# leggedrobotics/wild_visual_navigation

Measured on NVIDIA H100. Metric: frames/sec end-to-end (DINO feat + seg + MLP train-step) at 448x448, higher is better.
Workload: dtype bf16 operands / fp32 accumulate (ViT, STEGO head, per-pixel MLP); fp32 (k-means, train step)

## Files before the change

### include/wvn_b200.h

```cpp
#ifndef WVN_B200_H_
#define WVN_B200_H_

#include <stddef.h>
#include <stdint.h>

#ifdef __cplusplus
extern "C" {
#endif

typedef enum {
  WVN_STATUS_OK = 0,
  WVN_STATUS_INVALID = -1,
  WVN_STATUS_CUDA = -2,
  WVN_STATUS_NO_DEVICE = -3,
  WVN_STATUS_STATE = -4
} wvn_status;

const char* wvn_last_error(void);
int wvn_check_device(void);
int wvn_version(void);
long long wvn_launch_count(void);
void wvn_profile_enable(int category_mask);
int wvn_profile_collect(float* host_ms, long long* host_launches);

int wvn_gemm_bf16(const void* a_bf16, long long lda, const void* w_bf16, const float* bias, void* out, long long ldo,
                  int m, int n, int k, int out_kind, int act, int block_n, void* stream);

typedef struct {
  int m, n, k;
  int epi, act;
  int block_n;
  const void* a;
  long long lda;
  const void* w;
  const float* bias;
  void* out;
  long long ldo;
  const float* pos;
  int tokens_in, npad;
  int dim, heads;
  void* q_out;
  void* k_out;
  void* vt_out;
  int feat, trav_col;
  const void* x;
  long long ldx;
  float* trav;
  float* conf;
  float* loss_reco;
  const float* cg_mean;
  const float* cg_std;
  float cg_std_factor;
  int reverse_m;
  int registers;
  const void* residual;
  long long ldr;
} wvn_gemm_ex_args;
int wvn_gemm_bf16_ex(const wvn_gemm_ex_args* args, void* stream);

int wvn_attention_bf16(const void* q, const void* k, const void* vt, void* out, int batch, int heads, int npad,
                       int n_valid, float scale, void* stream);

int wvn_layernorm(const float* x, const float* gamma, const float* beta, void* out_bf16, long long rows, int dim,
                  float eps, void* stream);

typedef struct wvn_vit wvn_vit_t;

typedef struct {
  int image_size;
  int patch_size;
  int dim;
  int depth;
  int heads;
  int mlp_dim;
  int max_batch;
  int chunk;
  float ln_eps;
  int head_out;
  int registers;
} wvn_vit_config;

int wvn_vit_create(const wvn_vit_config* cfg, wvn_vit_t** out);
void wvn_vit_destroy(wvn_vit_t* h);

int wvn_vit_set_weight(wvn_vit_t* h, const char* name, const float* data, long long numel);

int wvn_vit_forward(wvn_vit_t* h, const float* img, int batch, int in_h, int in_w, int resized_h, int resized_w,
                    float* tokens_out, void* stream);

// ... 149 lines not shown
```

### wild_visual_navigation_b200/_C.py

```python
from __future__ import annotations

import ctypes
import os
from ctypes import POINTER, Structure, byref, c_char_p, c_float, c_int, c_longlong, c_size_t, c_void_p

import torch

_HERE = os.path.dirname(os.path.abspath(__file__))
LIB_PATH = os.environ.get("WVN_B200_LIB", os.path.join(_HERE, "libwvn_b200.so"))


class WvnError(RuntimeError):
    pass


class VitConfig(Structure):
    _fields_ = [
        ("image_size", c_int), ("patch_size", c_int), ("dim", c_int), ("depth", c_int), ("heads", c_int),
        ("mlp_dim", c_int), ("max_batch", c_int), ("chunk", c_int), ("ln_eps", c_float), ("head_out", c_int),
        ("registers", c_int),
    ]


class GemmExArgs(Structure):
    _fields_ = [
        ("m", c_int), ("n", c_int), ("k", c_int), ("epi", c_int), ("act", c_int), ("block_n", c_int),
        ("a", c_void_p), ("lda", c_longlong), ("w", c_void_p), ("bias", c_void_p), ("out", c_void_p), ("ldo", c_longlong),
        ("pos", c_void_p), ("tokens_in", c_int), ("npad", c_int), ("dim", c_int), ("heads", c_int),
        ("q_out", c_void_p), ("k_out", c_void_p), ("vt_out", c_void_p),
        ("feat", c_int), ("trav_col", c_int), ("x", c_void_p), ("ldx", c_longlong), ("trav", c_void_p),
        ("conf", c_void_p), ("loss_reco", c_void_p), ("cg_mean", c_void_p), ("cg_std", c_void_p),
        ("cg_std_factor", c_float), ("reverse_m", c_int), ("registers", c_int), ("residual", c_void_p), ("ldr", c_longlong),
    ]


class ResnetConfig(Structure):
    _fields_ = [("image_size", c_int), ("depth", c_int), ("max_batch", c_int)]


class TrainConfig(Structure):
    _fields_ = [
        ("w_trav", c_float), ("w_reco", c_float), ("std_factor", c_float), ("anomaly_balanced", c_int),
        ("lr", c_float), ("beta1", c_float), ("beta2", c_float), ("eps", c_float),
    ]


class FlowBuffers(Structure):
    _fields_ = [("mask0", c_void_p), ("mask1", c_void_p), ("p1", c_void_p), ("invp1", c_void_p), ("p3", c_void_p),
                ("invp3", c_void_p)]


_lib = None

_P, _I, _L, _F, _S = c_void_p, c_int, c_longlong, c_float, c_size_t
SIGNATURES = {
    "wvn_last_error": (c_char_p, []),
    "wvn_check_device": (_I, []),
    "wvn_version": (_I, []),
    "wvn_launch_count": (_L, []),
    "wvn_profile_enable": (None, [_I]),
    "wvn_profile_collect": (_I, [_P, _P]),
    "wvn_gemm_bf16": (_I, [_P, _L, _P, _P, _P, _L, _I, _I, _I, _I, _I, _I, _P]),
    "wvn_gemm_bf16_ex": (_I, [POINTER(GemmExArgs), _P]),
    "wvn_attention_bf16": (_I, [_P, _P, _P, _P, _I, _I, _I, _I, _F, _P]),
    "wvn_layernorm": (_I, [_P, _P, _P, _P, _L, _I, _F, _P]),
# ... 108 lines not shown
```

### wild_visual_navigation_b200/csrc/api.cu

```cuda
#include <cuda_bf16.h>

#include <stdio.h>
#include <stdlib.h>

#include <map>
#include <string>
#include <vector>

#include "../../include/wvn_b200.h"
#include "attention.h"
#include "dense_kernels.h"
#include "gemm.h"
#include "host_common.h"
#include "mlp_train.h"
#include "mlp_train_fused.h"
#include "pixel_head.h"
#include "resnet_kernels.h"
#include "segment_kernels.h"
#include "flow_train.h"
#include "footprint_kernels.h"
#include "slic_kernels.h"
#include "stego_kmeans.h"
#include "train_core.h"
#include "vit_kernels.h"
// ... 54 lines not shown
};

}

struct wvn_vit {
  wvn_vit_config cfg;
  int grid = 0, P = 0, t0 = 1, n_valid = 0, npad = 0, kpe = 0, kpe_ld = 0, chunk = 0;
  std::map<std::string, Weight> w;
  std::vector<DevBuf> owned;
  DevBuf x, xn, q, k, vt, attn, hid, ape, stage;
  DevBuf tok_bf16, head_hidden;
  DevBuf qkv_f32;
  bool precise = false;
  bool forwarded = false;
  int last_batch = 0;

  int add_weight(const std::string& name, long long numel, bool bf16, int cols = 0, int ld = 0) {
    DevBuf b;
    const long long stored = cols > 0 ? numel / cols * ld : numel;
    WVN_PROPAGATE(b.alloc(static_cast<size_t>(stored) * (bf16 ? 2 : 4)));
    owned.push_back(b);
    Weight wt;
    wt.p = b.p; wt.numel = numel; wt.bf16 = bf16; wt.cols = cols; wt.ld = ld;
    w[name] = wt;
    return WVN_OK;
  }
  template <class T>
  T* wp(const std::string& name) { return reinterpret_cast<T*>(w[name].p); }
};

extern "C" {

const char* wvn_last_error(void) { return last_error(); }
int wvn_version(void) { return 104; }

int wvn_check_device(void) {
  int n = 0;
  if (cudaGetDeviceCount(&n) != cudaSuccess || n == 0) return set_error(WVN_ERR_NO_DEVICE, "no CUDA device visible");
  int dev = 0;
  cudaGetDevice(&dev);
  int major = 0;
  cudaDeviceGetAttribute(&major, cudaDevAttrComputeCapabilityMajor, dev);
  int minor = 0;
  cudaDeviceGetAttribute(&minor, cudaDevAttrComputeCapabilityMinor, dev);
  if (major != 9 || minor != 0)
    return set_error(WVN_ERR_NO_DEVICE, "device %d has compute capability %d.%d, need 9.0 (sm_90a)", dev, major, minor);
  return WVN_OK;
}

long long wvn_launch_count(void) { return launch_count(); }
void wvn_profile_enable(int category_mask) { prof_enable(category_mask); }
int wvn_profile_collect(float* host_ms, long long* host_launches) {
  WVN_REQUIRE(host_ms && host_launches, "wvn_profile_collect: null argument");
  return prof_collect(host_ms, host_launches);
}

int wvn_gemm_bf16(const void* a, long long lda, const void* w, const float* bias, void* out, long long ldo, int m, int n,
                  int k, int out_kind, int act, int block_n, void* stream) {
  GemmArgs g;
  g.M = m; g.N = n; g.K = k;
  g.epi = out_kind == 0 ? EPI_BF16 : (out_kind == 1 ? EPI_F32 : EPI_RESID_F32);
  WVN_REQUIRE(out_kind >= 0 && out_kind <= 2, "wvn_gemm_bf16: out_kind %d", out_kind);
  g.act = act; g.bias = bias; g.out = out; g.ldo = ldo;
  return gemm_bf16(g, a, lda, w, block_n, S(stream));
}

int wvn_gemm_bf16_ex(const wvn_gemm_ex_args* x, void* stream) {
  WVN_REQUIRE(x, "wvn_gemm_bf16_ex: null argument");
  GemmArgs g;
  g.M = x->m; g.N = x->n; g.K = x->k; g.epi = x->epi; g.act = x->act;
  g.bias = x->bias; g.out = x->out; g.ldo = x->ldo;
  g.pos = x->pos; g.tokens_in = x->tokens_in; g.npad = x->npad;
  g.dim = x->dim; g.heads = x->heads; g.q = x->q_out; g.k = x->k_out; g.vt = x->vt_out;
  g.feat = x->feat; g.trav_col = x->trav_col; g.x = x->x; g.ldx = x->ldx; g.trav = x->trav; g.conf = x->conf;
  g.loss_reco = x->loss_reco; g.cg_mean = x->cg_mean; g.cg_std = x->cg_std; g.cg_std_factor = x->cg_std_factor;
  g.reverse_m = x->reverse_m; g.registers = x->registers;
  g.residual = x->residual; g.ldr = x->ldr;
  return gemm_bf16(g, x->a, x->lda, x->w, x->block_n, S(stream));
}

int wvn_attention_bf16(const void* q, const void* k, const void* vt, void* out, int batch, int heads, int npad,
                       int n_valid, float scale, void* stream) {
  AttnArgs a;
  a.batch = batch; a.heads = heads; a.npad = npad; a.n_valid = n_valid;
  a.scale_log2 = scale * 1.4426950408889634f;
  a.out = out; a.ldo = static_cast<long long>(heads) * 64;
  return attention_bf16(a, q, k, vt, S(stream));
}

int wvn_layernorm(const float* x, const float* gamma, const float* beta, void* out_bf16, long long rows, int dim,
                  float eps, void* stream) {
  LayerNormArgs a;
  a.rows = rows; a.dim = dim; a.eps = eps;
  return layernorm_rows(x, gamma, beta, out_bf16, nullptr, a, S(stream));
}

int wvn_vit_create(const wvn_vit_config* cfg, wvn_vit_t** out) {
  WVN_REQUIRE(cfg && out, "wvn_vit_create: null argument");
  WVN_PROPAGATE(wvn_check_device());
  WVN_REQUIRE(cfg->dim == 384 || cfg->dim == 768, "vit: dim %d unsupported (384, 768)", cfg->dim);
  WVN_REQUIRE(cfg->heads * 64 == cfg->dim, "vit: heads*64 must equal dim");
  WVN_REQUIRE(cfg->patch_size == 8 || cfg->patch_size == 14 || cfg->patch_size == 16, "vit: patch size %d unsupported",
              cfg->patch_size);
  WVN_REQUIRE(cfg->image_size >= cfg->patch_size, "vit: image size too small");
  WVN_REQUIRE(cfg->mlp_dim % 64 == 0 && cfg->depth > 0 && cfg->max_batch > 0, "vit: bad mlp_dim/depth/max_batch");
  WVN_REQUIRE(cfg->head_out % 64 == 0, "vit: head_out must be a multiple of 64");
  WVN_REQUIRE(cfg->registers >= 0, "vit: registers must be >= 0");
  WVN_REQUIRE(cfg->registers == 0 || cfg->head_out == 0, "vit: register tokens and a STEGO head cannot be combined");
  wvn_vit* h = new wvn_vit();
  h->cfg = *cfg;
// ... 129 lines not shown

static int vit_check_loaded(wvn_vit* h, bool need_head) {
  for (auto& kv : h->w) {
    const bool is_head = kv.first.rfind("stego.", 0) == 0;
    if (is_head && !need_head) continue;
    if (!kv.second.loaded) return set_error(WVN_ERR_STATE, "vit: weight '%s' was never set", kv.first.c_str());
  }
  return WVN_OK;
}

constexpr int kDefaultSubAttn = 1 << 30;

namespace {
int vit_forward_impl(wvn_vit_t* h, const void* img, bool u8_hwc, int batch, int in_h, int in_w, int resized_h, int resized_w,
                     float* tokens_out, void* stream, bool flip_tta = false);
}

int wvn_vit_forward_tta(wvn_vit_t* h, const float* img, int batch, int in_h, int in_w, int resized_h, int resized_w,
                        float* tokens_out, void* stream) {
  return vit_forward_impl(h, img, false, batch, in_h, in_w, resized_h, resized_w, tokens_out, stream, true);
}

int wvn_vit_forward(wvn_vit_t* h, const float* img, int batch, int in_h, int in_w, int resized_h, int resized_w,
                    float* tokens_out, void* stream) {
  return vit_forward_impl(h, img, false, batch, in_h, in_w, resized_h, resized_w, tokens_out, stream);
}

int wvn_vit_forward_u8(wvn_vit_t* h, const unsigned char* img_hwc, int batch, int in_h, int in_w, int resized_h,
                       int resized_w, float* tokens_out, void* stream) {
  return vit_forward_impl(h, img_hwc, true, batch, in_h, in_w, resized_h, resized_w, tokens_out, stream);
}

namespace {
int vit_forward_impl(wvn_vit_t* h, const void* img, bool u8_hwc, int src_batch, int in_h, int in_w, int resized_h, int resized_w,
                     float* tokens_out, void* stream, bool flip_tta) {
  const int batch = flip_tta ? 2 * src_batch : src_batch;
  WVN_REQUIRE(h && img, "wvn_vit_forward: null argument");
  WVN_REQUIRE(batch > 0 && batch <= h->cfg.max_batch, "wvn_vit_forward: batch %d outside (0, %d]", batch, h->cfg.max_batch);
  WVN_REQUIRE(resized_h >= h->cfg.image_size && resized_w >= h->cfg.image_size,
              "wvn_vit_forward: resized image %dx%d smaller than the crop %d", resized_h, resized_w, h->cfg.image_size);
  WVN_PROPAGATE(vit_check_loaded(h, false));
  cudaStream_t s = S(stream);
  const wvn_vit_config& c = h->cfg;
  const int D = c.dim;

  ImagePatchArgs ia;
  ia.in_h = in_h; ia.in_w = in_w; ia.patch = c.patch_size; ia.grid_h = h->grid; ia.grid_w = h->grid;
  ia.crop_top = static_cast<int>(lrintf((resized_h - c.image_size) / 2.0f));
  ia.crop_left = static_cast<int>(lrintf((resized_w - c.image_size) / 2.0f));
  ia.scale_y = static_cast<float>(in_h) / static_cast<float>(resized_h);
  ia.scale_x = static_cast<float>(in_w) / static_cast<float>(resized_w);

  for (int b0 = 0; b0 < batch; b0 += h->chunk) {
    const int nb = std::min(h->chunk, batch - b0);
    const int rows = nb * h->npad;
    float* x = reinterpret_cast<float*>(h->x.p);
    ia.batch = nb;
    ia.frame0 = b0; ia.src_frames = src_batch; ia.flip_from = flip_tta ? src_batch : (1 << 30);
    WVN_PROPAGATE(image_to_patches(img, u8_hwc, h->ape.p, ia, s));
    const float* reg = c.registers > 0 ? h->wp<float>("register_tokens") : nullptr;
    WVN_PROPAGATE(init_token_rows(x, h->wp<float>("cls_token"), h->wp<float>("pos_embed"), reg, c.registers, nb, h->npad,
                                  h->n_valid, D, s));
    {
      GemmArgs g;
      g.M = nb * h->P; g.N = D; g.K = h->kpe; g.epi = EPI_PATCH; g.bias = h->wp<float>("patch_embed.proj.bias");
      g.out = x; g.ldo = D; g.pos = h->wp<float>("pos_embed"); g.tokens_in = h->P; g.npad = h->npad;
      g.registers = c.registers;
      WVN_PROPAGATE(gemm_bf16(g, h->ape.p, h->kpe_ld, h->wp<void>("patch_embed.proj.weight"), 0, s));
    }
    LayerNormArgs la;
    la.rows = rows; la.dim = D; la.eps = c.ln_eps; la.npad = h->npad; la.n_valid = h->n_valid; la.row0 = h->t0;
    static int sub_env = -1;
    if (sub_env < 0) {
      const char* e = getenv("WVN_VIT_SUBCHUNK");
      sub_env = e ? atoi(e) : (1 << 30);
      if (sub_env < 1) sub_env = 1 << 30;
    }
// ... 8 lines not shown
    if (sub_attn_env < 0) {
      const char* e = getenv("WVN_VIT_SUB_ATTN");
      sub_attn_env = e ? atoi(e) : kDefaultSubAttn;
      if (sub_attn_env < 1) sub_attn_env = 1 << 30;
    }
    const int sub_a = std::min(sub_attn_env, nb);
    for (int l = 0; l < c.depth; ++l) {
      const std::string b = "blocks." + std::to_string(l) + ".";
      for (int s0 = 0; s0 < nb; s0 += sub_a) {
        const int ns = std::min(sub_a, nb - s0);
        const long long roff = static_cast<long long>(s0) * h->npad;
        LayerNormArgs ls = la;
        ls.rows = static_cast<long long>(ns) * h->npad;
        ls.reverse = next_dir();
        WVN_PROPAGATE(layernorm_rows(x + roff * D, h->wp<float>(b + "norm1.weight"), h->wp<float>(b + "norm1.bias"),
                                     xn + roff * D, nullptr, ls, s));
        if (h->precise) {
          GemmArgs g;
          float* qkv = reinterpret_cast<float*>(h->qkv_f32.p) + roff * 3 * D;
          g.M = ns * h->npad; g.N = 3 * D; g.K = D; g.epi = EPI_F32; g.bias = h->wp<float>(b + "attn.qkv.bias");
          g.out = qkv; g.ldo = 3 * D;
          WVN_PROPAGATE(gemm_bf16(g, xn + roff * D, D, h->wp<void>(b + "attn.qkv.weight"), 0, s));
          WVN_PROPAGATE(attention_f32_debug(qkv, attn + roff * D, ns, c.heads, h->npad, h->n_valid, D, 0.125f, s));
          continue;
        }
        GemmArgs g;
        g.M = ns * h->npad; g.N = 3 * D; g.K = D; g.epi = EPI_QKV; g.bias = h->wp<float>(b + "attn.qkv.bias");
        g.npad = h->npad; g.dim = D; g.heads = c.heads;
        const long long hoff = static_cast<long long>(s0) * c.heads * h->npad * 64;
        g.q = reinterpret_cast<__nv_bfloat16*>(h->q.p) + hoff;
        g.k = reinterpret_cast<__nv_bfloat16*>(h->k.p) + hoff;
        g.vt = reinterpret_cast<__nv_bfloat16*>(h->vt.p) + hoff;
        g.reverse_m = next_dir();
        WVN_PROPAGATE(gemm_bf16(g, xn + roff * D, D, h->wp<void>(b + "attn.qkv.weight"), 0, s));
        AttnArgs a;
        a.batch = ns; a.heads = c.heads; a.npad = h->npad; a.n_valid = h->n_valid;
        a.scale_log2 = 0.125f * 1.4426950408889634f;
        a.out = attn + roff * D; a.ldo = D;
        a.reverse = next_dir();
        WVN_PROPAGATE(attention_bf16(a, g.q, g.k, g.vt, s));
      }
      for (int s0 = 0; s0 < nb; s0 += sub) {
        const int ns = std::min(sub, nb - s0);
        const long long roff = static_cast<long long>(s0) * h->npad;
        const int srows = ns * h->npad;
        LayerNormArgs ls = la;
        ls.rows = srows;
        {
          GemmArgs g;
          g.M = srows; g.N = D; g.K = D; g.epi = EPI_RESID_F32; g.bias = h->wp<float>(b + "attn.proj.bias");
          g.out = x + roff * D; g.ldo = D;
          g.reverse_m = next_dir();
          WVN_PROPAGATE(gemm_bf16(g, attn + roff * D, D, h->wp<void>(b + "attn.proj.weight"), 0, s));
        }
        ls.reverse = next_dir();
        WVN_PROPAGATE(layernorm_rows(x + roff * D, h->wp<float>(b + "norm2.weight"), h->wp<float>(b + "norm2.bias"),
                                     xn + roff * D, nullptr, ls, s));
        {
          GemmArgs g;
          g.M = srows; g.N = c.mlp_dim; g.K = D; g.epi = EPI_BF16; g.act = ACT_GELU;
          g.bias = h->wp<float>(b + "mlp.fc1.bias"); g.out = h->hid.p; g.ldo = c.mlp_dim;
          g.reverse_m = next_dir();
          WVN_PROPAGATE(gemm_bf16(g, xn + roff * D, D, h->wp<void>(b + "mlp.fc1.weight"), 0, s));
        }
        {
          GemmArgs g;
          g.M = srows; g.N = D; g.K = c.mlp_dim; g.epi = EPI_RESID_F32; g.bias = h->wp<float>(b + "mlp.fc2.bias");
          g.out = x + roff * D; g.ldo = D;
          g.reverse_m = next_dir();
          WVN_PROPAGATE(gemm_bf16(g, h->hid.p, c.mlp_dim, h->wp<void>(b + "mlp.fc2.weight"), 0, s));
        }
      }
    }
    __nv_bfloat16* tok_bf = reinterpret_cast<__nv_bfloat16*>(h->tok_bf16.p) + static_cast<long long>(b0) * h->npad * D;
    float* tok_f = tokens_out ? tokens_out + static_cast<long long>(b0) * h->P * D : nullptr;
    la.reverse = next_dir();
    WVN_PROPAGATE(layernorm_rows(x, h->wp<float>("norm.weight"), h->wp<float>("norm.bias"), tok_bf, tok_f, la, s));
  }
  h->forwarded = true;
  h->last_batch = batch;
  return WVN_OK;
}
}

int wvn_vit_stego_head(wvn_vit_t* h, int batch, float* out, void* stream) {
  WVN_REQUIRE(h && out, "wvn_vit_stego_head: null argument");
  WVN_REQUIRE(h->cfg.head_out > 0, "wvn_vit_stego_head: handle was created without a head");
  WVN_REQUIRE(h->forwarded && batch == h->last_batch, "wvn_vit_stego_head: call wvn_vit_forward with the same batch first");
  WVN_PROPAGATE(vit_check_loaded(h, true));
  cudaStream_t s = S(stream);
  const int D = h->cfg.dim, rows = batch * h->npad, HO = h->cfg.head_out;
  GemmArgs g;
  g.M = rows; g.N = D; g.K = D; g.epi = EPI_BF16; g.act = ACT_RELU; g.bias = h->wp<float>("stego.hidden.bias");
  g.out = h->head_hidden.p; g.ldo = D;
  WVN_PROPAGATE(gemm_bf16(g, h->tok_bf16.p, D, h->wp<void>("stego.hidden.weight"), 0, s));
  GemmArgs a;
  a.M = rows; a.N = HO; a.K = D; a.epi = EPI_F32; a.bias = h->wp<float>("stego.head_a.bias"); a.out = out; a.ldo = HO;
  WVN_PROPAGATE(gemm_bf16(a, h->tok_bf16.p, D, h->wp<void>("stego.head_a.weight"), 0, s));
  GemmArgs b;
  b.M = rows; b.N = HO; b.K = D; b.epi = EPI_RESID_F32; b.bias = nullptr; b.out = out; b.ldo = HO;
  WVN_PROPAGATE(gemm_bf16(b, h->head_hidden.p, D, h->wp<void>("stego.head_b.weight"), 0, s));
  return WVN_OK;
}
// ... 830 lines not shown
```

### wild_visual_navigation_b200/csrc/gemm.h

```cpp
#pragma once

#include <cuda_runtime.h>

namespace wvn {

enum GemmEpilogue : int {
  EPI_BF16 = 0,
  EPI_F32 = 1,
  EPI_RESID_F32 = 2,
  EPI_PATCH = 3,
  EPI_QKV = 4,
  EPI_MLP_HEAD = 5,
  EPI_BF16_RESID = 6,
};

enum GemmAct : int { ACT_NONE = 0, ACT_RELU = 1, ACT_GELU = 2 };

struct GemmArgs {
  int M = 0, N = 0, K = 0;
  int epi = EPI_BF16, act = ACT_NONE;
  const float* bias = nullptr;
  void* out = nullptr;
  long long ldo = 0;
  const float* pos = nullptr;
  int tokens_in = 0;
  int registers = 0;
  int npad = 0;
  int dim = 0, heads = 0;
  void* q = nullptr;
  void* k = nullptr;
  void* vt = nullptr;
  int feat = 0;
  int trav_col = 0;
  const void* x = nullptr;
  long long ldx = 0;
  float* trav = nullptr;
  float* conf = nullptr;
  float* loss_reco = nullptr;
  const float* cg_mean = nullptr;
  const float* cg_std = nullptr;
  float cg_std_factor = 0.5f;
  const void* residual = nullptr;
  long long ldr = 0;
  int max_ctas = 0;
  int reverse_m = 0;
};

int pick_block_n(int N);

inline long long gemm_w_pitch(int K) { return (static_cast<long long>(K) + 7) / 8 * 8; }

int gemm_bf16(const GemmArgs& args, const void* A, long long lda, const void* W, int block_n, cudaStream_t stream);

}
```

### wild_visual_navigation_b200/csrc/gemm_wgmma.cu

```cuda
#include <stdlib.h>

#include <algorithm>

#include "common.cuh"
#include "gemm.h"
#include "host_common.h"

namespace wvn {

namespace {

constexpr int BM = 64;
constexpr int BK = 64;
constexpr int kConsumerWarps = 8;
constexpr int kNumThreads = 128 + kConsumerWarps * 32;
constexpr int kMaxSmemBytes = 227 * 1024;
constexpr int kMaxStages = 8;
constexpr int kFixedSmemBytes = 1024  + 1024 ;
constexpr int kSliceCols = 32;
constexpr int kResidMaxBlockN = 192;

template <bool ROW_OWNER>
struct TileIter {
  int num_m, num_n, m_blk, n_blk, lin;
  __device__ TileIter(int nm, int nn) : num_m(nm), num_n(nn), m_blk(0), n_blk(0), lin(0) {
    if (ROW_OWNER) { m_blk = blockIdx.x; n_blk = 0; }
    else { lin = blockIdx.x; m_blk = lin / num_n; n_blk = lin % num_n; }
  }
  __device__ bool valid() const { return m_blk < num_m; }
  __device__ void next() {
    if (ROW_OWNER) { if (++n_blk == num_n) { n_blk = 0; m_blk += gridDim.x; } }
    else { lin += gridDim.x; m_blk = lin / num_n; n_blk = lin % num_n; }
  }
};

template <int EPI>
constexpr bool kStaged = EPI == EPI_BF16 || EPI == EPI_F32 || EPI == EPI_RESID_F32 || EPI == EPI_QKV || EPI == EPI_BF16_RESID;

template <int BN, int EPI>
struct GemmCfg {
  static constexpr uint32_t kABytes = BM * BK * 2;
  static constexpr uint32_t kBBytes = BN * BK * 2;
  static constexpr uint32_t kStageBytes = kABytes + kBBytes;
  static constexpr uint32_t kSliceBytes = BM * kSliceCols * ((EPI == EPI_F32 || EPI == EPI_RESID_F32) ? 4 : 2);
  static constexpr uint32_t kStagingBytes = kStaged<EPI> ? 2 * 2 * kSliceBytes : 0;
  static constexpr int kStagesRaw = (kMaxSmemBytes - kFixedSmemBytes - kStagingBytes) / kStageBytes;
  static constexpr int kStages = kStagesRaw > kMaxStages ? kMaxStages : kStagesRaw;
  static constexpr uint32_t kSmemBytes = kStages * kStageBytes + kStagingBytes + kFixedSmemBytes;
  static constexpr int kN128 = BN / 128;
  static constexpr int kN64 = (BN % 128) / 64;
  static constexpr int kN32 = (BN % 64) / 32;
};

__device__ __forceinline__ float gelu_erf_fast(float x) {
  const float t = fminf(fabsf(x), 5.5f);
  float p = fmaf(-0.0003865310864f, t, 0.006509808358f);
  p = fmaf(p, t, -0.05048002675f);
  p = fmaf(p, t, -0.4613505006f);
  p = fmaf(p, t, -1.150225043f);
  p = fmaf(p, t, -1.00010848f);
  float e;
  asm("ex2.approx.ftz.f32 %0, %1;" : "=f"(e) : "f"(p));
  return fmaf(-t, e, fmaxf(x, 0.f));
}

template <int ACT>
__device__ __forceinline__ float activate(float v) {
  if (ACT == ACT_RELU) return fmaxf(v, 0.f);
  if (ACT == ACT_GELU) return gelu_erf_fast(v);
  return v;
}

template <int EPI, int ACT, int NREG>
__device__ __forceinline__ void epilogue_frag(const GemmArgs& args, const float (&d)[NREG], const int row0,
// ... 81 lines not shown
        }
        const float v0 = activate<ACT>(a0), v1 = activate<ACT>(a1);
        if (EPI == EPI_F32 || EPI == EPI_RESID_F32) {
          sts64(buf + r * 128 + ((((2 * js + (q >> 1)) ^ (r & 7))) << 4) + (q & 1) * 8, v0, v1);
        } else if (EPI == EPI_QKV && which == 2) {
          const int dd = 8 * js + 2 * q;
          const uint32_t t = 2 * r;
          sts16(buf + dd * 128 + (((t >> 4) ^ (dd & 7)) << 4) + (t & 15), __float2bfloat16_rn(v0));
          sts16(buf + (dd + 1) * 128 + (((t >> 4) ^ ((dd + 1) & 7)) << 4) + (t & 15), __float2bfloat16_rn(v1));
        } else {
          sts32(buf + r * 64 + ((js ^ ((r >> 1) & 3)) << 4) + q * 4, pack_bf16x2(v0, v1));
        }
      }
    }
    fence_proxy_async_smem();
    named_bar_sync(bar_id, 128);
    if (leader) {
      if (EPI == EPI_BF16 || EPI == EPI_F32 || EPI == EPI_BF16_RESID) {
        tma_store_2d(tm0, buf, col, row_tile);
      } else if (EPI == EPI_RESID_F32) {
        tma_reduce_add_2d(tm0, buf, col, row_tile);
      } else if (EPI == EPI_QKV) {
        const int frame = row_tile / args.npad;
        const int tok0 = row_tile - frame * args.npad;
        const int bh = frame * args.heads + (within >> 6);
        if (which < 2) tma_store_2d(which == 0 ? tm0 : tm1, buf, within & 63, bh * args.npad + tok0);
        else tma_store_2d(tm2, buf, tok0, bh * 64 + (within & 63));
      }
      tma_store_commit();
    }
  }
}

template <int BN, int EPI, int ACT>
__global__ void __launch_bounds__(kNumThreads, 1)
gemm_bf16_kernel(const __grid_constant__ CUtensorMap tmap_a, const __grid_constant__ CUtensorMap tmap_b,
                 const __grid_constant__ CUtensorMap tmap_c0, const __grid_constant__ CUtensorMap tmap_c1,
                 const __grid_constant__ CUtensorMap tmap_c2, const GemmArgs args) {
  using Cfg = GemmCfg<BN, EPI>;
  constexpr int STAGES = Cfg::kStages;

  extern __shared__ uint8_t smem_raw[];
  uint8_t* smem = reinterpret_cast<uint8_t*>((reinterpret_cast<uintptr_t>(smem_raw) + 1023) & ~uintptr_t(1023));
  uint8_t* smem_b = smem;
  uint8_t* smem_a = smem + STAGES * Cfg::kBBytes;
  uint8_t* smem_c = smem_a + STAGES * Cfg::kABytes;
  uint64_t* bars = reinterpret_cast<uint64_t*>(smem_c + Cfg::kStagingBytes);
  uint64_t* full_bar = bars;
  uint64_t* empty_bar = bars + kMaxStages;

  const int warp = threadIdx.x >> 5;
  const int lane = threadIdx.x & 31;

  const int num_m = (args.M + BM - 1) / BM;
  const int num_n = args.N / BN;
  const int num_k = (args.K + BK - 1) / BK;
  constexpr bool ROW_OWNER = (EPI == EPI_MLP_HEAD);

  if (threadIdx.x == 0) {
    tma_prefetch_desc(&tmap_a);
    tma_prefetch_desc(&tmap_b);
    for (int i = 0; i < kMaxStages; ++i) {
      mbar_init(&full_bar[i], 1);
      mbar_init(&empty_bar[i], kConsumerWarps / 2);
    }
    fence_mbar_init();
  }
  __syncthreads();

  if (warp < 4) {
    setmaxnreg_dec<40>();
    if (warp == 0) {
      int stage = 0;
      uint32_t phase = 0;
      for (TileIter<ROW_OWNER> it(num_m, num_n); it.valid(); it.next()) {
        const int m_eff = args.reverse_m ? num_m - 1 - it.m_blk : it.m_blk;
        for (int kb = 0; kb < num_k; ++kb) {
          mbar_wait(&empty_bar[stage], phase ^ 1);
          if (elect_one_sync()) {
            mbar_arrive_expect_tx(&full_bar[stage], Cfg::kStageBytes);
            tma_load_2d(&tmap_a, &full_bar[stage], smem_a + stage * Cfg::kABytes, kb * BK, m_eff * BM);
            tma_load_2d(&tmap_b, &full_bar[stage], smem_b + stage * Cfg::kBBytes, kb * BK, it.n_blk * BN);
          }
          __syncwarp();
          if (++stage == STAGES) { stage = 0; phase ^= 1; }
        }
      }
    }
  } else {
    setmaxnreg_inc<232>();
    const int cwarp = warp - 4;
    const int wg = cwarp >> 2;
    const int row_local = (cwarp & 3) * 16 + (lane >> 2);
    const bool leader = (threadIdx.x & 127) == 0;
    const uint32_t staging = smem_u32(smem_c) + wg * 2 * Cfg::kSliceBytes;
    if (kStaged<EPI> && leader) {
      tma_prefetch_desc(&tmap_c0);
      if (EPI == EPI_QKV) {
        tma_prefetch_desc(&tmap_c1);
        tma_prefetch_desc(&tmap_c2);
      }
    }
    if (wg == 1) named_bar_arrive(1, 256);
    float acc128[Cfg::kN128 > 0 ? Cfg::kN128 : 1][64];
    float acc64[32];
    float acc32[16];
    float head_partial[2] = {0.f, 0.f};
    int stage = 0;
    uint32_t phase = 0;
    int unit = 0;
    for (TileIter<ROW_OWNER> it(num_m, num_n); it.valid(); it.next()) {
      const bool unit_end = !ROW_OWNER || it.n_blk == num_n - 1;
      if ((unit & 1) != wg) {
        for (int kb = 0; kb < num_k; ++kb)
          if (++stage == STAGES) { stage = 0; phase ^= 1; }
        if (unit_end) ++unit;
        continue;
      }
      if (!ROW_OWNER || it.n_blk == 0) named_bar_sync(1 + wg, 256);
      int prev_stage = 0;
      for (int kb = 0; kb < num_k; ++kb) {
        mbar_wait(&full_bar[stage], phase);
        const uint64_t desc_a = make_sw128_kmajor_desc(smem_u32(smem_a + stage * Cfg::kABytes));
        const uint32_t b_addr = smem_u32(smem_b + stage * Cfg::kBBytes);
#pragma unroll
        for (int c = 0; c < Cfg::kN128; ++c) wgmma_fence_regs(acc128[c]);
        if (Cfg::kN64) wgmma_fence_regs(acc64);
        if (Cfg::kN32) wgmma_fence_regs(acc32);
        wgmma_fence();
#pragma unroll
        for (int k = 0; k < BK / 16; ++k) {
          const uint32_t accumulate = (kb | k) != 0 ? 1u : 0u;
#pragma unroll
          for (int c = 0; c < Cfg::kN128; ++c)
            wgmma_m64n128k16_ss(acc128[c], desc_a + 2 * k, make_sw128_kmajor_desc(b_addr + c * 128 * 128) + 2 * k, accumulate);
          if (Cfg::kN64)
            wgmma_m64n64k16_ss(acc64, desc_a + 2 * k, make_sw128_kmajor_desc(b_addr + Cfg::kN128 * 128 * 128) + 2 * k, accumulate);
          if (Cfg::kN32)
            wgmma_m64n32k16_ss(acc32, desc_a + 2 * k,
                               make_sw128_kmajor_desc(b_addr + (Cfg::kN128 * 128 + Cfg::kN64 * 64) * 128) + 2 * k, accumulate);
        }
        wgmma_commit();
        if (kb > 0) {
          wgmma_wait<1>();
          if (lane == 0) mbar_arrive(&empty_bar[prev_stage]);
        }
        prev_stage = stage;
        if (++stage == STAGES) { stage = 0; phase ^= 1; }
      }
      if (unit_end && (ROW_OWNER ? it.m_blk + static_cast<int>(gridDim.x) < num_m : it.lin + static_cast<int>(gridDim.x) < num_m * num_n))
        named_bar_arrive(2 - wg, 256);
      wgmma_wait<0>();
#pragma unroll
      for (int c = 0; c < Cfg::kN128; ++c) wgmma_fence_regs(acc128[c]);
      if (Cfg::kN64) wgmma_fence_regs(acc64);
      if (Cfg::kN32) wgmma_fence_regs(acc32);
      if (lane == 0) mbar_arrive(&empty_bar[prev_stage]);

      const int m_eff = args.reverse_m ? num_m - 1 - it.m_blk : it.m_blk;
      const int row_tile = m_eff * BM;
      const int col0 = it.n_blk * BN;
      if (kStaged<EPI>) {
        const int bar_id = 3 + wg;
#pragma unroll
        for (int c = 0; c < Cfg::kN128; ++c)
          store_frag<EPI, ACT>(args, &tmap_c0, &tmap_c1, &tmap_c2, acc128[c], row_tile, col0 + c * 128, row_local, lane,
                               leader, bar_id, staging, Cfg::kSliceBytes, 4 * c);
        if (Cfg::kN64)
          store_frag<EPI, ACT>(args, &tmap_c0, &tmap_c1, &tmap_c2, acc64, row_tile, col0 + Cfg::kN128 * 128, row_local,
                               lane, leader, bar_id, staging, Cfg::kSliceBytes, 4 * Cfg::kN128);
        if (Cfg::kN32)
          store_frag<EPI, ACT>(args, &tmap_c0, &tmap_c1, &tmap_c2, acc32, row_tile, col0 + Cfg::kN128 * 128 + Cfg::kN64 * 64,
                               row_local, lane, leader, bar_id, staging, Cfg::kSliceBytes, 4 * Cfg::kN128 + 2 * Cfg::kN64);
      } else {
        const int row0 = row_tile + row_local;
#pragma unroll
        for (int c = 0; c < Cfg::kN128; ++c)
          epilogue_frag<EPI, ACT>(args, acc128[c], row0, col0 + c * 128, lane, head_partial);
        if (Cfg::kN64) epilogue_frag<EPI, ACT>(args, acc64, row0, col0 + Cfg::kN128 * 128, lane, head_partial);
        if (Cfg::kN32) epilogue_frag<EPI, ACT>(args, acc32, row0, col0 + Cfg::kN128 * 128 + Cfg::kN64 * 64, lane, head_partial);
      }

      if (EPI == EPI_MLP_HEAD && it.n_blk == num_n - 1) {
#pragma unroll
        for (int h = 0; h < 2; ++h) {
          float s = head_partial[h];
          s += __shfl_xor_sync(0xffffffffu, s, 1);
          s += __shfl_xor_sync(0xffffffffu, s, 2);
          head_partial[h] = 0.f;
          const int row = row_tile + row_local + 8 * h;
          if ((lane & 3) == 0 && row < args.M) {
            const float loss = s / static_cast<float>(args.feat);
            const float mean = __ldg(args.cg_mean), sd = __ldg(args.cg_std);
            const float shifted = mean + sd * args.cg_std_factor;
            const float lo = fmaxf(shifted - sd, 0.f);
            const float hi = shifted + sd;
            const float xc = fminf(fmaxf(loss, lo), hi);
            args.conf[row] = 1.f - (xc - lo) / (hi - lo);
            if (args.loss_reco != nullptr) args.loss_reco[row] = loss;
          }
        }
      }
      if (unit_end) ++unit;
    }
    if (kStaged<EPI> && leader) tma_store_wait_all<0>();
  }
}

template <int BN, int EPI, int ACT>
int launch_gemm(const GemmArgs& a, const CUtensorMap& ta, const CUtensorMap& tb, const CUtensorMap (&tc)[3],
                cudaStream_t stream) {
  using Cfg = GemmCfg<BN, EPI>;
  static_assert(Cfg::kStages >= 2, "tile too wide for the shared-memory budget");
  auto kern = gemm_bf16_kernel<BN, EPI, ACT>;
  static bool attr_set = false;
  if (!attr_set) {
    WVN_CHECK_CUDA(cudaFuncSetAttribute(kern, cudaFuncAttributeMaxDynamicSharedMemorySize, kMaxSmemBytes));
    attr_set = true;
  }
  const int num_m = (a.M + BM - 1) / BM, num_n = a.N / BN;
  const int num_tiles = (EPI == EPI_MLP_HEAD) ? num_m : num_m * num_n;
  int grid = sm_count();
  if (a.max_ctas > 0 && a.max_ctas < grid) grid = a.max_ctas;
  if (grid > num_tiles) grid = num_tiles;
  prof_begin(PROF_GEMM, stream);
  kern<<<grid, kNumThreads, Cfg::kSmemBytes, stream>>>(ta, tb, tc[0], tc[1], tc[2], a);
  prof_end(PROF_GEMM, stream);
  WVN_CHECK_LAUNCH("gemm_bf16_kernel");
  return WVN_OK;
}

template <int BN>
int dispatch_epi(const GemmArgs& a, const CUtensorMap& ta, const CUtensorMap& tb, const CUtensorMap (&tc)[3],
                 cudaStream_t s) {
  switch (a.epi) {
    case EPI_BF16:
      if (a.act == ACT_NONE) return launch_gemm<BN, EPI_BF16, ACT_NONE>(a, ta, tb, tc, s);
      if (a.act == ACT_RELU) return launch_gemm<BN, EPI_BF16, ACT_RELU>(a, ta, tb, tc, s);
      if (a.act == ACT_GELU) return launch_gemm<BN, EPI_BF16, ACT_GELU>(a, ta, tb, tc, s);
      break;
    case EPI_F32:
      if (a.act == ACT_NONE) return launch_gemm<BN, EPI_F32, ACT_NONE>(a, ta, tb, tc, s);
      break;
    case EPI_RESID_F32:
      if (a.act == ACT_NONE) return launch_gemm<BN, EPI_RESID_F32, ACT_NONE>(a, ta, tb, tc, s);
      break;
    case EPI_PATCH:
      if (a.act == ACT_NONE) return launch_gemm<BN, EPI_PATCH, ACT_NONE>(a, ta, tb, tc, s);
      break;
    case EPI_QKV:
      if (a.act == ACT_NONE) return launch_gemm<BN, EPI_QKV, ACT_NONE>(a, ta, tb, tc, s);
      break;
    case EPI_MLP_HEAD:
      if (a.act == ACT_NONE) return launch_gemm<BN, EPI_MLP_HEAD, ACT_NONE>(a, ta, tb, tc, s);
      break;
    case EPI_BF16_RESID:
      if constexpr (BN <= kResidMaxBlockN) {
        if (a.act == ACT_NONE) return launch_gemm<BN, EPI_BF16_RESID, ACT_NONE>(a, ta, tb, tc, s);
        if (a.act == ACT_RELU) return launch_gemm<BN, EPI_BF16_RESID, ACT_RELU>(a, ta, tb, tc, s);
      }
      break;
  }
  return set_error(WVN_ERR_INVALID, "gemm: unsupported epilogue/activation combination (%d, %d)", a.epi, a.act);
}

}

int pick_block_n(int N) {
  if (N % 256 == 0) return 256;
  if (N % 224 == 0) return 224;
  if (N % 192 == 0) return 192;
  if (N % 128 == 0) return 128;
  if (N % 64 == 0) return 64;
  return 0;
}

int gemm_bf16(const GemmArgs& a, const void* A, long long lda, const void* W, int block_n, cudaStream_t stream) {
  WVN_REQUIRE(a.M > 0 && a.N > 0 && a.K > 0, "gemm: empty problem (M=%d N=%d K=%d)", a.M, a.N, a.K);
  WVN_REQUIRE(lda >= a.K, "gemm: lda=%lld is smaller than K=%d", lda, a.K);
  if (block_n == 0) {
    block_n = pick_block_n(a.N);
    if (a.epi == EPI_BF16_RESID && block_n > kResidMaxBlockN) block_n = a.N % 192 == 0 ? 192 : (a.N % 128 == 0 ? 128 : 64);
  }
  WVN_REQUIRE(a.epi != EPI_BF16_RESID || block_n <= kResidMaxBlockN, "gemm: the residual epilogue takes block_n <= %d",
              kResidMaxBlockN);
  WVN_REQUIRE(block_n == 64 || block_n == 128 || block_n == 192 || block_n == 224 || block_n == 256,
              "gemm: bad block_n %d", block_n);
  WVN_REQUIRE(a.N % block_n == 0, "gemm: N=%d must be a multiple of block_n=%d (pad the weights)", a.N, block_n);
  if (a.epi == EPI_MLP_HEAD)
    WVN_REQUIRE(a.feat > 0 && a.trav_col % 32 == 0 && a.trav_col >= a.feat && a.trav_col < a.N && a.x != nullptr &&
                    a.trav != nullptr && a.conf != nullptr && a.cg_mean != nullptr && a.cg_std != nullptr &&
                    a.ldx % 8 == 0 && a.ldx >= a.trav_col,
                "gemm: bad MLP-head epilogue arguments (feat=%d trav_col=%d N=%d)", a.feat, a.trav_col, a.N);
  if (a.epi == EPI_QKV)
    WVN_REQUIRE(a.dim % 64 == 0 && a.N == 3 * a.dim && a.heads * 64 == a.dim && a.npad % 8 == 0 && a.npad % BM == 0 &&
                    a.M % a.npad == 0,
                "gemm: bad QKV epilogue geometry (dim=%d heads=%d npad=%d N=%d M=%d)", a.dim, a.heads, a.npad, a.N, a.M);
  if (a.epi == EPI_PATCH)
    WVN_REQUIRE(a.tokens_in > 0 && a.registers >= 0 && 1 + a.registers + a.tokens_in <= a.npad,
                "gemm: bad patch-embed epilogue geometry (tokens_in=%d registers=%d npad=%d)", a.tokens_in, a.registers,
                a.npad);
  if (a.epi == EPI_F32 || a.epi == EPI_RESID_F32) WVN_REQUIRE(a.ldo % 4 == 0, "gemm: fp32 output pitch must be a multiple of 4");
  if (a.epi == EPI_BF16 || a.epi == EPI_BF16_RESID) WVN_REQUIRE(a.ldo % 8 == 0, "gemm: bf16 output pitch must be a multiple of 8");
  if (a.epi == EPI_BF16_RESID)
    WVN_REQUIRE(a.residual != nullptr && a.ldr >= a.N && a.ldr % 2 == 0,
                "gemm: the residual epilogue needs a bf16 residual with an even pitch ldr >= N (ldr=%lld N=%d)", a.ldr, a.N);
  CUtensorMap ta, tb, tc[3] = {};
  WVN_PROPAGATE(make_tmap_bf16_2d(&ta, A, a.K, a.M, static_cast<uint64_t>(lda) * 2, BK, BM));
  WVN_PROPAGATE(make_tmap_bf16_2d(&tb, W, a.K, a.N, static_cast<uint64_t>(gemm_w_pitch(a.K)) * 2, BK, block_n));
  if (a.epi == EPI_BF16 || a.epi == EPI_BF16_RESID)
    WVN_PROPAGATE(make_tmap_2d(&tc[0], a.out, 2, a.N, a.M, static_cast<uint64_t>(a.ldo) * 2, kSliceCols, BM, 64));
  if (a.epi == EPI_F32 || a.epi == EPI_RESID_F32)
    WVN_PROPAGATE(make_tmap_2d(&tc[0], a.out, 4, a.N, a.M, static_cast<uint64_t>(a.ldo) * 4, kSliceCols, BM, 128));
  if (a.epi == EPI_QKV) {
    const uint64_t bh = static_cast<uint64_t>(a.M / a.npad) * a.heads;
    WVN_PROPAGATE(make_tmap_2d(&tc[0], a.q, 2, 64, bh * a.npad, 128, kSliceCols, BM, 64));
    WVN_PROPAGATE(make_tmap_2d(&tc[1], a.k, 2, 64, bh * a.npad, 128, kSliceCols, BM, 64));
    WVN_PROPAGATE(make_tmap_2d(&tc[2], a.vt, 2, a.npad, bh * 64, static_cast<uint64_t>(a.npad) * 2, BM, kSliceCols, 128));
  }
  switch (block_n) {
    case 64: return dispatch_epi<64>(a, ta, tb, tc, stream);
    case 128: return dispatch_epi<128>(a, ta, tb, tc, stream);
    case 192: return dispatch_epi<192>(a, ta, tb, tc, stream);
    case 224: return dispatch_epi<224>(a, ta, tb, tc, stream);
    case 256: return dispatch_epi<256>(a, ta, tb, tc, stream);
  }
  return set_error(WVN_ERR_INVALID, "gemm: unreachable");
}

}
```

Measured before the change: 974.9.

## Add cooperative two-warpgroup GEMM schedule for ViT QKV and MLP projections

Adds a cooperative schedule where both consumer warpgroups share one 2*BM-row tile and a single B tile per stage, instead of ping-pong alternating whole tiles. The ViT QKV, fc1 and fc2 GEMMs now request this schedule with explicit block_n choices. The aim is to halve B-operand traffic per output row and raise arithmetic intensity. In exchange, larger A stages reduce pipeline depth, there are fewer tiles (more wave quantization risk), and the epilogue no longer overlaps with the other warpgroup's mainloop.

```diff
diff --git a/include/wvn_b200.h b/include/wvn_b200.h
--- a/include/wvn_b200.h
+++ b/include/wvn_b200.h
@@ -55,6 +55,7 @@
   int registers;
   const void* residual;
   long long ldr;
+  int schedule;
 } wvn_gemm_ex_args;
 int wvn_gemm_bf16_ex(const wvn_gemm_ex_args* args, void* stream);
 
diff --git a/wild_visual_navigation_b200/_C.py b/wild_visual_navigation_b200/_C.py
--- a/wild_visual_navigation_b200/_C.py
+++ b/wild_visual_navigation_b200/_C.py
@@ -31,6 +31,7 @@
         ("feat", c_int), ("trav_col", c_int), ("x", c_void_p), ("ldx", c_longlong), ("trav", c_void_p),
         ("conf", c_void_p), ("loss_reco", c_void_p), ("cg_mean", c_void_p), ("cg_std", c_void_p),
         ("cg_std_factor", c_float), ("reverse_m", c_int), ("registers", c_int), ("residual", c_void_p), ("ldr", c_longlong),
+        ("schedule", c_int),
     ]
 
 
diff --git a/wild_visual_navigation_b200/csrc/api.cu b/wild_visual_navigation_b200/csrc/api.cu
--- a/wild_visual_navigation_b200/csrc/api.cu
+++ b/wild_visual_navigation_b200/csrc/api.cu
@@ -110,7 +110,7 @@
 extern "C" {
 
 const char* wvn_last_error(void) { return last_error(); }
-int wvn_version(void) { return 104; }
+int wvn_version(void) { return 105; }
 
 int wvn_check_device(void) {
   int n = 0;
@@ -153,7 +153,7 @@
   g.feat = x->feat; g.trav_col = x->trav_col; g.x = x->x; g.ldx = x->ldx; g.trav = x->trav; g.conf = x->conf;
   g.loss_reco = x->loss_reco; g.cg_mean = x->cg_mean; g.cg_std = x->cg_std; g.cg_std_factor = x->cg_std_factor;
   g.reverse_m = x->reverse_m; g.registers = x->registers;
-  g.residual = x->residual; g.ldr = x->ldr;
+  g.residual = x->residual; g.ldr = x->ldr; g.schedule = x->schedule;
   return gemm_bf16(g, x->a, x->lda, x->w, x->block_n, S(stream));
 }
 
@@ -349,6 +349,14 @@
 }
 
 namespace {
+int vit_coop(GemmArgs& g, int preferred) {
+  g.schedule = SCHED_COOP;
+  for (int bn : {preferred, 256, 192, 128})
+    if (g.N % bn == 0) return bn;
+  g.schedule = SCHED_PINGPONG;
+  return 0;
+}
+
 int vit_forward_impl(wvn_vit_t* h, const void* img, bool u8_hwc, int src_batch, int in_h, int in_w, int resized_h, int resized_w,
                      float* tokens_out, void* stream, bool flip_tta) {
   const int batch = flip_tta ? 2 * src_batch : src_batch;
@@ -360,6 +368,7 @@
   cudaStream_t s = S(stream);
   const wvn_vit_config& c = h->cfg;
   const int D = c.dim;
+  const int QKV_BN = 192, FC1_BN = 192, FC2_BN = D <= 384 ? 128 : 256;
 
   ImagePatchArgs ia;
   ia.in_h = in_h; ia.in_w = in_w; ia.patch = c.patch_size; ia.grid_h = h->grid; ia.grid_w = h->grid;
@@ -434,7 +443,8 @@
         g.k = reinterpret_cast<__nv_bfloat16*>(h->k.p) + hoff;
         g.vt = reinterpret_cast<__nv_bfloat16*>(h->vt.p) + hoff;
         g.reverse_m = next_dir();
-        WVN_PROPAGATE(gemm_bf16(g, xn + roff * D, D, h->wp<void>(b + "attn.qkv.weight"), 0, s));
+        const int qkv_bn = vit_coop(g, QKV_BN);
+        WVN_PROPAGATE(gemm_bf16(g, xn + roff * D, D, h->wp<void>(b + "attn.qkv.weight"), qkv_bn, s));
         AttnArgs a;
         a.batch = ns; a.heads = c.heads; a.npad = h->npad; a.n_valid = h->n_valid;
         a.scale_log2 = 0.125f * 1.4426950408889634f;
@@ -463,14 +473,16 @@
           g.M = srows; g.N = c.mlp_dim; g.K = D; g.epi = EPI_BF16; g.act = ACT_GELU;
           g.bias = h->wp<float>(b + "mlp.fc1.bias"); g.out = h->hid.p; g.ldo = c.mlp_dim;
           g.reverse_m = next_dir();
-          WVN_PROPAGATE(gemm_bf16(g, xn + roff * D, D, h->wp<void>(b + "mlp.fc1.weight"), 0, s));
+          const int fc1_bn = vit_coop(g, FC1_BN);
+          WVN_PROPAGATE(gemm_bf16(g, xn + roff * D, D, h->wp<void>(b + "mlp.fc1.weight"), fc1_bn, s));
         }
         {
           GemmArgs g;
           g.M = srows; g.N = D; g.K = c.mlp_dim; g.epi = EPI_RESID_F32; g.bias = h->wp<float>(b + "mlp.fc2.bias");
           g.out = x + roff * D; g.ldo = D;
           g.reverse_m = next_dir();
-          WVN_PROPAGATE(gemm_bf16(g, h->hid.p, c.mlp_dim, h->wp<void>(b + "mlp.fc2.weight"), 0, s));
+          const int fc2_bn = vit_coop(g, FC2_BN);
+          WVN_PROPAGATE(gemm_bf16(g, h->hid.p, c.mlp_dim, h->wp<void>(b + "mlp.fc2.weight"), fc2_bn, s));
         }
       }
     }
diff --git a/wild_visual_navigation_b200/csrc/gemm.h b/wild_visual_navigation_b200/csrc/gemm.h
--- a/wild_visual_navigation_b200/csrc/gemm.h
+++ b/wild_visual_navigation_b200/csrc/gemm.h
@@ -15,6 +15,8 @@
 };
 
 enum GemmAct : int { ACT_NONE = 0, ACT_RELU = 1, ACT_GELU = 2 };
+
+enum GemmSchedule : int { SCHED_PINGPONG = 0, SCHED_COOP = 1 };
 
 struct GemmArgs {
   int M = 0, N = 0, K = 0;
@@ -44,6 +46,7 @@
   long long ldr = 0;
   int max_ctas = 0;
   int reverse_m = 0;
+  int schedule = SCHED_PINGPONG;
 };
 
 int pick_block_n(int N);
diff --git a/wild_visual_navigation_b200/csrc/gemm_wgmma.cu b/wild_visual_navigation_b200/csrc/gemm_wgmma.cu
--- a/wild_visual_navigation_b200/csrc/gemm_wgmma.cu
+++ b/wild_visual_navigation_b200/csrc/gemm_wgmma.cu
@@ -37,9 +37,12 @@
 template <int EPI>
 constexpr bool kStaged = EPI == EPI_BF16 || EPI == EPI_F32 || EPI == EPI_RESID_F32 || EPI == EPI_QKV || EPI == EPI_BF16_RESID;
 
-template <int BN, int EPI>
+template <int BN, int EPI, int SCHED>
 struct GemmCfg {
-  static constexpr uint32_t kABytes = BM * BK * 2;
+  static constexpr bool kCoop = SCHED == SCHED_COOP;
+  static constexpr int kTileRows = kCoop ? 2 * BM : BM;
+  static constexpr uint32_t kHalfABytes = BM * BK * 2;
+  static constexpr uint32_t kABytes = kTileRows * BK * 2;
   static constexpr uint32_t kBBytes = BN * BK * 2;
   static constexpr uint32_t kStageBytes = kABytes + kBBytes;
   static constexpr uint32_t kSliceBytes = BM * kSliceCols * ((EPI == EPI_F32 || EPI == EPI_RESID_F32) ? 4 : 2);
@@ -187,13 +190,16 @@
   }
 }
 
-template <int BN, int EPI, int ACT>
+template <int BN, int EPI, int ACT, int SCHED>
 __global__ void __launch_bounds__(kNumThreads, 1)
 gemm_bf16_kernel(const __grid_constant__ CUtensorMap tmap_a, const __grid_constant__ CUtensorMap tmap_b,
                  const __grid_constant__ CUtensorMap tmap_c0, const __grid_constant__ CUtensorMap tmap_c1,
                  const __grid_constant__ CUtensorMap tmap_c2, const GemmArgs args) {
-  using Cfg = GemmCfg<BN, EPI>;
+  using Cfg = GemmCfg<BN, EPI, SCHED>;
   constexpr int STAGES = Cfg::kStages;
+  constexpr bool COOP = Cfg::kCoop;
+  constexpr int TM = Cfg::kTileRows;
+  static_assert(!COOP || kStaged<EPI>, "the cooperative schedule serves the staged epilogues only");
 
   extern __shared__ uint8_t smem_raw[];
   uint8_t* smem = reinterpret_cast<uint8_t*>((reinterpret_cast<uintptr_t>(smem_raw) + 1023) & ~uintptr_t(1023));
@@ -207,7 +213,7 @@
   const int warp = threadIdx.x >> 5;
   const int lane = threadIdx.x & 31;
 
-  const int num_m = (args.M + BM - 1) / BM;
+  const int num_m = (args.M + TM - 1) / TM;
   const int num_n = args.N / BN;
   const int num_k = (args.K + BK - 1) / BK;
   constexpr bool ROW_OWNER = (EPI == EPI_MLP_HEAD);
@@ -217,7 +223,7 @@
     tma_prefetch_desc(&tmap_b);
     for (int i = 0; i < kMaxStages; ++i) {
       mbar_init(&full_bar[i], 1);
-      mbar_init(&empty_bar[i], kConsumerWarps / 2);
+      mbar_init(&empty_bar[i], COOP ? kConsumerWarps : kConsumerWarps / 2);
     }
     fence_mbar_init();
   }
@@ -230,11 +236,15 @@
       uint32_t phase = 0;
       for (TileIter<ROW_OWNER> it(num_m, num_n); it.valid(); it.next()) {
         const int m_eff = args.reverse_m ? num_m - 1 - it.m_blk : it.m_blk;
+        const int row0 = m_eff * TM;
+        const bool lower = COOP && row0 + BM < args.M;
         for (int kb = 0; kb < num_k; ++kb) {
           mbar_wait(&empty_bar[stage], phase ^ 1);
           if (elect_one_sync()) {
-            mbar_arrive_expect_tx(&full_bar[stage], Cfg::kStageBytes);
-            tma_load_2d(&tmap_a, &full_bar[stage], smem_a + stage * Cfg::kABytes, kb * BK, m_eff * BM);
+            mbar_arrive_expect_tx(&full_bar[stage], Cfg::kBBytes + (lower ? 2 : 1) * Cfg::kHalfABytes);
+            tma_load_2d(&tmap_a, &full_bar[stage], smem_a + stage * Cfg::kABytes, kb * BK, row0);
+            if (lower)
+              tma_load_2d(&tmap_a, &full_bar[stage], smem_a + stage * Cfg::kABytes + Cfg::kHalfABytes, kb * BK, row0 + BM);
             tma_load_2d(&tmap_b, &full_bar[stage], smem_b + stage * Cfg::kBBytes, kb * BK, it.n_blk * BN);
           }
           __syncwarp();
@@ -256,7 +266,10 @@
         tma_prefetch_desc(&tmap_c2);
       }
     }
-    if (wg == 1) named_bar_arrive(1, 256);
+    const int lag = max(1, min(num_k, STAGES) / 2);
+    if (!COOP && wg == 1) named_bar_arrive(1, 256);
+    if (COOP && wg == 1) named_bar_sync(1, 256);
+    bool first = true;
     float acc128[Cfg::kN128 > 0 ? Cfg::kN128 : 1][64];
     float acc64[32];
     float acc32[16];
@@ -266,17 +279,20 @@
     int unit = 0;
     for (TileIter<ROW_OWNER> it(num_m, num_n); it.valid(); it.next()) {
       const bool unit_end = !ROW_OWNER || it.n_blk == num_n - 1;
-      if ((unit & 1) != wg) {
-        for (int kb = 0; kb < num_k; ++kb)
-          if (++stage == STAGES) { stage = 0; phase ^= 1; }
-        if (unit_end) ++unit;
-        continue;
-      }
-      if (!ROW_OWNER || it.n_blk == 0) named_bar_sync(1 + wg, 256);
+      if (!COOP) {
+        if ((unit & 1) != wg) {
+          for (int kb = 0; kb < num_k; ++kb)
+            if (++stage == STAGES) { stage = 0; phase ^= 1; }
+          if (unit_end) ++unit;
+          continue;
+        }
+        if (!ROW_OWNER || it.n_blk == 0) named_bar_sync(1 + wg, 256);
+      }
       int prev_stage = 0;
       for (int kb = 0; kb < num_k; ++kb) {
         mbar_wait(&full_bar[stage], phase);
-        const uint64_t desc_a = make_sw128_kmajor_desc(smem_u32(smem_a + stage * Cfg::kABytes));
+        const uint64_t desc_a =
+            make_sw128_kmajor_desc(smem_u32(smem_a + stage * Cfg::kABytes + (COOP ? wg * Cfg::kHalfABytes : 0)));
         const uint32_t b_addr = smem_u32(smem_b + stage * Cfg::kBBytes);
 #pragma unroll
         for (int c = 0; c < Cfg::kN128; ++c) wgmma_fence_regs(acc128[c]);
@@ -302,8 +318,11 @@
         }
         prev_stage = stage;
         if (++stage == STAGES) { stage = 0; phase ^= 1; }
-      }
-      if (unit_end && (ROW_OWNER ? it.m_blk + static_cast<int>(gridDim.x) < num_m : it.lin + static_cast<int>(gridDim.x) < num_m * num_n))
+        if (COOP && first && wg == 0 && kb == lag - 1) named_bar_arrive(1, 256);
+      }
+      first = false;
+      if (!COOP && unit_end &&
+          (ROW_OWNER ? it.m_blk + static_cast<int>(gridDim.x) < num_m : it.lin + static_cast<int>(gridDim.x) < num_m * num_n))
         named_bar_arrive(2 - wg, 256);
       wgmma_wait<0>();
 #pragma unroll
@@ -313,9 +332,10 @@
       if (lane == 0) mbar_arrive(&empty_bar[prev_stage]);
 
       const int m_eff = args.reverse_m ? num_m - 1 - it.m_blk : it.m_blk;
-      const int row_tile = m_eff * BM;
+      const int row_tile = m_eff * TM + (COOP ? wg * BM : 0);
       const int col0 = it.n_blk * BN;
       if (kStaged<EPI>) {
+        if (row_tile >= args.M) continue;
         const int bar_id = 3 + wg;
 #pragma unroll
         for (int c = 0; c < Cfg::kN128; ++c)
@@ -362,18 +382,18 @@
   }
 }
 
-template <int BN, int EPI, int ACT>
+template <int BN, int EPI, int ACT, int SCHED>
 int launch_gemm(const GemmArgs& a, const CUtensorMap& ta, const CUtensorMap& tb, const CUtensorMap (&tc)[3],
                 cudaStream_t stream) {
-  using Cfg = GemmCfg<BN, EPI>;
+  using Cfg = GemmCfg<BN, EPI, SCHED>;
   static_assert(Cfg::kStages >= 2, "tile too wide for the shared-memory budget");
-  auto kern = gemm_bf16_kernel<BN, EPI, ACT>;
+  auto kern = gemm_bf16_kernel<BN, EPI, ACT, SCHED>;
   static bool attr_set = false;
   if (!attr_set) {
     WVN_CHECK_CUDA(cudaFuncSetAttribute(kern, cudaFuncAttributeMaxDynamicSharedMemorySize, kMaxSmemBytes));
     attr_set = true;
   }
-  const int num_m = (a.M + BM - 1) / BM, num_n = a.N / BN;
+  const int num_m = (a.M + Cfg::kTileRows - 1) / Cfg::kTileRows, num_n = a.N / BN;
   const int num_tiles = (EPI == EPI_MLP_HEAD) ? num_m : num_m * num_n;
   int grid = sm_count();
   if (a.max_ctas > 0 && a.max_ctas < grid) grid = a.max_ctas;
@@ -385,38 +405,50 @@
   return WVN_OK;
 }
 
-template <int BN>
+template <int BN, int SCHED>
 int dispatch_epi(const GemmArgs& a, const CUtensorMap& ta, const CUtensorMap& tb, const CUtensorMap (&tc)[3],
                  cudaStream_t s) {
+  constexpr bool kPing = SCHED == SCHED_PINGPONG;
   switch (a.epi) {
     case EPI_BF16:
-      if (a.act == ACT_NONE) return launch_gemm<BN, EPI_BF16, ACT_NONE>(a, ta, tb, tc, s);
-      if (a.act == ACT_RELU) return launch_gemm<BN, EPI_BF16, ACT_RELU>(a, ta, tb, tc, s);
-      if (a.act == ACT_GELU) return launch_gemm<BN, EPI_BF16, ACT_GELU>(a, ta, tb, tc, s);
+      if (a.act == ACT_NONE) return launch_gemm<BN, EPI_BF16, ACT_NONE, SCHED>(a, ta, tb, tc, s);
+      if (a.act == ACT_RELU) return launch_gemm<BN, EPI_BF16, ACT_RELU, SCHED>(a, ta, tb, tc, s);
+      if (a.act == ACT_GELU) return launch_gemm<BN, EPI_BF16, ACT_GELU, SCHED>(a, ta, tb, tc, s);
       break;
     case EPI_F32:
-      if (a.act == ACT_NONE) return launch_gemm<BN, EPI_F32, ACT_NONE>(a, ta, tb, tc, s);
+      if (a.act == ACT_NONE) return launch_gemm<BN, EPI_F32, ACT_NONE, SCHED>(a, ta, tb, tc, s);
       break;
     case EPI_RESID_F32:
-      if (a.act == ACT_NONE) return launch_gemm<BN, EPI_RESID_F32, ACT_NONE>(a, ta, tb, tc, s);
+      if (a.act == ACT_NONE) return launch_gemm<BN, EPI_RESID_F32, ACT_NONE, SCHED>(a, ta, tb, tc, s);
       break;
     case EPI_PATCH:
-      if (a.act == ACT_NONE) return launch_gemm<BN, EPI_PATCH, ACT_NONE>(a, ta, tb, tc, s);
+      if constexpr (kPing)
+        if (a.act == ACT_NONE) return launch_gemm<BN, EPI_PATCH, ACT_NONE, SCHED>(a, ta, tb, tc, s);
       break;
     case EPI_QKV:
-      if (a.act == ACT_NONE) return launch_gemm<BN, EPI_QKV, ACT_NONE>(a, ta, tb, tc, s);
+      if (a.act == ACT_NONE) return launch_gemm<BN, EPI_QKV, ACT_NONE, SCHED>(a, ta, tb, tc, s);
       break;
     case EPI_MLP_HEAD:
-      if (a.act == ACT_NONE) return launch_gemm<BN, EPI_MLP_HEAD, ACT_NONE>(a, ta, tb, tc, s);
+      if constexpr (kPing)
+        if (a.act == ACT_NONE) return launch_gemm<BN, EPI_MLP_HEAD, ACT_NONE, SCHED>(a, ta, tb, tc, s);
       break;
     case EPI_BF16_RESID:
-      if constexpr (BN <= kResidMaxBlockN) {
-        if (a.act == ACT_NONE) return launch_gemm<BN, EPI_BF16_RESID, ACT_NONE>(a, ta, tb, tc, s);
-        if (a.act == ACT_RELU) return launch_gemm<BN, EPI_BF16_RESID, ACT_RELU>(a, ta, tb, tc, s);
-      }
-      break;
-  }
-  return set_error(WVN_ERR_INVALID, "gemm: unsupported epilogue/activation combination (%d, %d)", a.epi, a.act);
+      if constexpr (kPing && BN <= kResidMaxBlockN) {
+        if (a.act == ACT_NONE) return launch_gemm<BN, EPI_BF16_RESID, ACT_NONE, SCHED>(a, ta, tb, tc, s);
+        if (a.act == ACT_RELU) return launch_gemm<BN, EPI_BF16_RESID, ACT_RELU, SCHED>(a, ta, tb, tc, s);
+      }
+      break;
+  }
+  return set_error(WVN_ERR_INVALID, "gemm: unsupported epilogue/activation/schedule combination (%d, %d, %d)", a.epi,
+                   a.act, a.schedule);
+}
+
+template <int BN>
+int dispatch_sched(const GemmArgs& a, const CUtensorMap& ta, const CUtensorMap& tb, const CUtensorMap (&tc)[3],
+                   cudaStream_t s) {
+  if constexpr (BN == 128 || BN == 192 || BN == 256)
+    if (a.schedule == SCHED_COOP) return dispatch_epi<BN, SCHED_COOP>(a, ta, tb, tc, s);
+  return dispatch_epi<BN, SCHED_PINGPONG>(a, ta, tb, tc, s);
 }
 
 }
@@ -442,6 +474,12 @@
   WVN_REQUIRE(block_n == 64 || block_n == 128 || block_n == 192 || block_n == 224 || block_n == 256,
               "gemm: bad block_n %d", block_n);
   WVN_REQUIRE(a.N % block_n == 0, "gemm: N=%d must be a multiple of block_n=%d (pad the weights)", a.N, block_n);
+  WVN_REQUIRE(a.schedule == SCHED_PINGPONG || a.schedule == SCHED_COOP, "gemm: bad schedule %d", a.schedule);
+  if (a.schedule == SCHED_COOP)
+    WVN_REQUIRE((a.epi == EPI_BF16 || a.epi == EPI_F32 || a.epi == EPI_RESID_F32 || a.epi == EPI_QKV) &&
+                    (block_n == 128 || block_n == 192 || block_n == 256),
+                "gemm: the cooperative schedule takes epilogues 0, 1, 2, 4 and block_n 128, 192 or 256 (epi=%d block_n=%d)",
+                a.epi, block_n);
   if (a.epi == EPI_MLP_HEAD)
     WVN_REQUIRE(a.feat > 0 && a.trav_col % 32 == 0 && a.trav_col >= a.feat && a.trav_col < a.N && a.x != nullptr &&
                     a.trav != nullptr && a.conf != nullptr && a.cg_mean != nullptr && a.cg_std != nullptr &&
@@ -474,11 +512,11 @@
     WVN_PROPAGATE(make_tmap_2d(&tc[2], a.vt, 2, a.npad, bh * 64, static_cast<uint64_t>(a.npad) * 2, BM, kSliceCols, 128));
   }
   switch (block_n) {
-    case 64: return dispatch_epi<64>(a, ta, tb, tc, stream);
-    case 128: return dispatch_epi<128>(a, ta, tb, tc, stream);
-    case 192: return dispatch_epi<192>(a, ta, tb, tc, stream);
-    case 224: return dispatch_epi<224>(a, ta, tb, tc, stream);
-    case 256: return dispatch_epi<256>(a, ta, tb, tc, stream);
+    case 64: return dispatch_sched<64>(a, ta, tb, tc, stream);
+    case 128: return dispatch_sched<128>(a, ta, tb, tc, stream);
+    case 192: return dispatch_sched<192>(a, ta, tb, tc, stream);
+    case 224: return dispatch_sched<224>(a, ta, tb, tc, stream);
+    case 256: return dispatch_sched<256>(a, ta, tb, tc, stream);
   }
   return set_error(WVN_ERR_INVALID, "gemm: unreachable");
 }
```

Measured after the change: 995.4, median of 6. 1.02x the previous value.
